# NVIDIAGameWorks/RayTracingDenoiser

Hardware: AMD Instinct MI355X
Metric: Mpixels/s REBLUR_DIFFUSE_SPECULAR @1440p (higher is better)
Workload: dtype f32

## Files before the change

raytracingdenoiser_amd/csrc/hip/kernels_reblur_spatial.hip:

```cpp
#include "passes.h"
#include "reblur_device.h"

namespace nrdhip {

constexpr int TILE_X = 32;
constexpr int TILE_Y = 8;

__global__ __launch_bounds__(256) void ReblurClassifyTilesKernel(Plane viewZ, Plane tiles, float viewZScale, float denoisingRange, int tilesPerRow, int tileRows) {
    const int wave = threadIdx.x >> 6, lane = threadIdx.x & 63;
    const int tileIndex = blockIdx.x * 4 + wave;
    if (tileIndex >= tilesPerRow * tileRows)
        return;
    const int tx = tileIndex % tilesPerRow, ty = tileIndex / tilesPerRow;
    const int x = tx * 16 + (lane & 3) * 4, y = ty * 16 + (lane >> 2);

    bool allSky = true;
    if (y < viewZ.h && x + 3 < viewZ.w) {
        float4 z = *(const float4*)TexelPtr<const float>(viewZ, x, y);
        allSky = Abs(z.x * viewZScale) > denoisingRange && Abs(z.y * viewZScale) > denoisingRange && Abs(z.z * viewZScale) > denoisingRange && Abs(z.w * viewZScale) > denoisingRange;
    } else {
        for (int i = 0; i < 4; i++) {
            float z = InBounds(viewZ, x + i, y) ? LoadR32F(viewZ, x + i, y) : 0.0f;
            allSky = allSky && Abs(z * viewZScale) > denoisingRange;
        }
// ... 24 lines not shown
    float viewZ, roughness, materialID, NoV, frustumSize;
    float3 N, Nv, Xv, Vv;
    float4 rotator;
    float2 data1;
    float3 geo;
    int cbX0, cbX1;
    float2 wc;
};

struct TapGuides {
    float w;
    float3 Ns, Xvs;
    float NvXvs;
    float roughnessS, materialIDs, zs;
    int2 ts;
    float2 uv;
};

template <int FR, bool NEED_ROUGHNESS>
NRD_D TapGuides FetchTapGuidesFullRect(const ReblurCB& c, const SpatialCtx& s, float2 k, const NormalRoughnessGuide& gIn_Normal_Roughness, const Plane& gIn_ViewPos, bool compareMaterials) {
    TapGuides t;
    const float2 rectSize = ToF2(c.gRectSize), rectSizeInv = ToF2(c.gRectSizeInv);
    const float cxf = __builtin_amdgcn_fmed3f(k.x, 0.0f, rectSize.x - 1.0f), cyf = __builtin_amdgcn_fmed3f(k.y, 0.0f, rectSize.y - 1.0f);
    t.w = (cxf == k.x && cyf == k.y) ? 1.0f : 0.0f;
    t.ts = make_int2((int)cxf, (int)cyf);
    const bool materials = FR == 1 && compareMaterials;
    uint32_t bits = 0u;
    {
        const uint32_t offset = TexelOffset(gIn_ViewPos, t.ts.x, t.ts.y, 16u, true);
        const float4 g = *(const float4*)(gIn_ViewPos.ptr + offset);
        t.Ns = Xyz(g);
        t.zs = g.w;
        if (NEED_ROUGHNESS || FR == 1)
            bits = *(const uint32_t*)(gIn_Normal_Roughness.word.ptr + (offset >> 2));
    }
    const float2 uvc = (k + 0.5f) * rectSizeInv;
    t.Xvs = ReconstructViewPosition(uvc, ToF4(c.gFrustum), t.zs, 0.0f);
    t.NvXvs = t.zs * (k.x * s.geo.x + (k.y * s.geo.y + s.geo.z));
    t.materialIDs = 0.0f;
    if (materials)
        t.materialIDs = DecodedMaterialID(bits);
    t.roughnessS = NEED_ROUGHNESS ? DecodedRoughness(bits) : 0.0f;
    t.uv = k;
    return t;
}

template <SpatialMode MODE, bool CB, int FR, bool NEED_ROUGHNESS>
NRD_D TapGuides FetchTapGuides(const ReblurCB& c, const SpatialCtx& s, float2 uv, const Plane& gIn_Signal, const Plane& gIn_ViewZ, const NormalRoughnessGuide& gIn_Normal_Roughness, const Plane& gIn_ViewPos,
    uint32_t checkerboardMode, uint32_t n, bool compareMaterials) {
    const float2 rectSize = ToF2(c.gRectSize), rectSizeInv = ToF2(c.gRectSizeInv);
    uv = Floor(uv * rectSize);
    if (FR)
        return FetchTapGuidesFullRect<FR, NEED_ROUGHNESS>(c, s, uv, gIn_Normal_Roughness, gIn_ViewPos, compareMaterials);
    TapGuides t;
    uv = uv + 0.5f;
    if (MODE == PRE_BLUR && CB)
        uv = ApplyCheckerboardShift(uv, checkerboardMode, n, c.gFrameIndex);
    const float2 k = uv - 0.5f;
    uv = uv * rectSizeInv;
    const float2 resolutionScale = ToF2(c.gResolutionScale);
    const float2 uvMax = resolutionScale - ToF2(c.gResourceSizeInv) * 0.5f;
    float2 uvScaled = F2(Min(uv.x * resolutionScale.x, uvMax.x), Min(uv.y * resolutionScale.y, uvMax.y));
    const int2 tz = NearestTexel(gIn_ViewZ, uvScaled);
    t.ts = tz;
    if (MODE == PRE_BLUR && CB && checkerboardMode != 2)
        t.ts = NearestTexel(gIn_Signal, F2(uvScaled.x * 0.5f, uvScaled.y));
    t.zs = UnpackViewZ(c, LoadR32F(gIn_ViewZ, tz.x, tz.y));
    float4 Ns = LoadDecodedNormalRoughness(gIn_Normal_Roughness, tz.x, tz.y, t.materialIDs);
// ... 1 lines not shown
    t.roughnessS = Ns.w;
    t.Xvs = ReconstructViewPosition(uv, ToF4(c.gFrustum), t.zs, NRD_ORTHO_MODE(c));
    t.NvXvs = t.zs * (k.x * s.geo.x + (k.y * s.geo.y + s.geo.z));
    t.w = IsInScreenNearest(uv);
    t.uv = uv;
    return t;
}

template <bool PERF>
NRD_D float PoissonGaussianWeight(int n) {
    if (PERF)
        return n < 3 ? REBLUR_GAUSSIAN_WEIGHT_Z1 : REBLUR_GAUSSIAN_WEIGHT_Z03;
    return n < 4 ? REBLUR_GAUSSIAN_WEIGHT_Z1 : REBLUR_GAUSSIAN_WEIGHT_Z05;
}

template <SpatialMode MODE, bool PERF, int KIND, bool SH, bool CB, int FR>
NRD_D typename ReblurSignal<KIND>::type DiffuseSpatialFilterTaps(const ReblurCB& c, const SpatialCtx& s, typename ReblurSignal<KIND>::type diff, const Plane& gIn_Diff, const Plane& gIn_ViewZ,
    const NormalRoughnessGuide& gIn_Normal_Roughness, const Plane& gIn_ViewPos, float4& diffSh, const Plane& gIn_DiffSh, float& sum) {
    typedef ReblurSignal<KIND> Sig;
    constexpr bool OCC = KIND == SIGNAL_OCCLUSION;
    typedef typename Sig::type S;

    float fractionScale = 1.0f, radiusScale = 1.0f;
    if (MODE == PRE_BLUR)
        fractionScale = REBLUR_PRE_BLUR_FRACTION_SCALE;
    else if (MODE == BLUR)
        fractionScale = REBLUR_BLUR_FRACTION_SCALE;
    else {
        radiusScale = REBLUR_POST_BLUR_RADIUS_SCALE;
        fractionScale = REBLUR_POST_BLUR_FRACTION_SCALE;
    }
// ... 24 lines not shown
    float2 hitDistanceWeightParams = GetHitDistanceWeightParams(ExtractHitDist(diff), diffNonLinearAccumSpeed);
    float minHitDistWeight = c.gMinHitDistanceWeight * fractionScale;
    if (MODE != PRE_BLUR && !OCC)
        minHitDistWeight *= Sqrt(diffNonLinearAccumSpeed);

    const float2 rectSizeInv = ToF2(c.gRectSizeInv);

    float2 skew = F2(1.0f, 1.0f);
    if (MODE != PRE_BLUR) {
        skew = Lerp(F2(1.0f - Abs(s.Nv.x), 1.0f - Abs(s.Nv.y)), F2(1.0f, 1.0f), s.NoV);
        skew = Div(skew, Max(skew.x, skew.y));
    }
    skew = skew * (rectSizeInv * blurRadius);
    float4 scaledRotator = ScaleRotator(s.rotator, skew);
    const bool compareMaterials = FR != 2 && c.gDiffMinMaterial < 3.0f;

#pragma unroll
    for (int n = 0; n < (PERF ? 6 : 8); n++) {
        float3 offset = PERF ? F3(g_Special6[n][0], g_Special6[n][1], g_Special6[n][2]) : F3(g_Special8[n][0], g_Special8[n][1], g_Special8[n][2]);
        const float2 uvTap = s.pixelUv + RotateVector(scaledRotator, F2(offset.x, offset.y));
        TapGuides t = FetchTapGuides<MODE, CB, FR, false>(c, s, uvTap, gIn_Diff, gIn_ViewZ, gIn_Normal_Roughness, gIn_ViewPos, c.gDiffCheckerboard, (uint32_t)n, compareMaterials);
        const int2 ts = t.ts;

        float angle = AcosApprox(Dot(s.N, t.Ns));

        float w = t.w;
        w *= ComputeWeight(t.NvXvs, geometryWeightParams.x, geometryWeightParams.y);
        if (compareMaterials)
            w *= CompareMaterials(s.materialID, t.materialIDs, c.gDiffMinMaterial) ? 1.0f : 0.0f;
        w *= ComputeWeight(angle, normalWeightParam, 0.0f);

        S smp = Sig::LoadOrZero(gIn_Diff, ts.x, ts.y, w == 0.0f);

        w *= Lerp(minHitDistWeight, 1.0f, ComputeExponentialWeight(ExtractHitDist(smp), hitDistanceWeightParams.x, hitDistanceWeightParams.y));
        w *= PoissonGaussianWeight<PERF>(n);

        sum += w;
        diff = Mad(smp, w, diff);
        if (SH) {
            float4 sh = LoadRGBA16F(gIn_DiffSh, ts.x, ts.y);
            sh = Select(w == 0.0f, F4(0.0f), sh);
            diffSh = Mad(sh, w, diffSh);
        }
    }

    float invSum = PositiveRcp(sum);
    if (SH)
        diffSh = diffSh * invSum;
    return diff * invSum;
}

template <SpatialMode MODE, bool PERF, int KIND, bool SH, bool CB, int FR>
NRD_D typename ReblurSignal<KIND>::type DiffuseSpatialFilter(const ReblurCB& c, const SpatialCtx& s, typename ReblurSignal<KIND>::type diff, const Plane& gIn_Diff, const Plane& gIn_ViewZ,
    const NormalRoughnessGuide& gIn_Normal_Roughness, const Plane& gIn_ViewPos, float4& diffSh, const Plane& gIn_DiffSh, float sum) {
    typedef ReblurSignal<KIND> Sig;
    typedef typename Sig::type S;
    if (!(MODE == PRE_BLUR && c.gDiffPrepassBlurRadius == 0.0f))
        diff = DiffuseSpatialFilterTaps<MODE, PERF, KIND, SH, CB, FR>(c, s, diff, gIn_Diff, gIn_ViewZ, gIn_Normal_Roughness, gIn_ViewPos, diffSh, gIn_DiffSh, sum);
    if (MODE == PRE_BLUR && CB && sum == 0.0f) {
        S s0 = Select(s.wc.x == 0.0f, Sig::Zero(), Sig::Load(gIn_Diff, s.cbX0, s.py));
        S s1 = Select(s.wc.y == 0.0f, Sig::Zero(), Sig::Load(gIn_Diff, s.cbX1, s.py));
        diff = s0 * s.wc.x + s1 * s.wc.y;
        if (SH) {
            float4 sh0 = Select(s.wc.x == 0.0f, F4(0.0f), LoadRGBA16F(gIn_DiffSh, s.cbX0, s.py));
            float4 sh1 = Select(s.wc.y == 0.0f, F4(0.0f), LoadRGBA16F(gIn_DiffSh, s.cbX1, s.py));
            diffSh = sh0 * s.wc.x + sh1 * s.wc.y;
        }
    }
    return diff;
}

template <SpatialMode MODE, bool PERF, int KIND, bool SH, bool CB, int FR>
NRD_D typename ReblurSignal<KIND>::type SpecularSpatialFilterTaps(const ReblurCB& c, const SpatialCtx& s, typename ReblurSignal<KIND>::type spec, const Plane& gIn_Spec, const Plane& gIn_ViewZ,
    const NormalRoughnessGuide& gIn_Normal_Roughness, const Plane& gIn_ViewPos, const Plane& gOut_SpecHitDistForTracking, float4& specSh, const Plane& gIn_SpecSh, float& sum) {
    typedef ReblurSignal<KIND> Sig;
    constexpr bool OCC = KIND == SIGNAL_OCCLUSION;
    typedef typename Sig::type S;
    float smc = GetSpecMagicCurve(s.roughness);

    RngHash rng;
    if (MODE == PRE_BLUR)
        rng.Initialize((uint32_t)s.px, (uint32_t)s.py, c.gFrameIndex);

    float fractionScale = 1.0f, radiusScale = 1.0f;
    if (MODE == PRE_BLUR)
        fractionScale = REBLUR_PRE_BLUR_FRACTION_SCALE;
    else if (MODE == BLUR)
// ... 34 lines not shown
    }
    blurRadius *= radiusScale;
    blurRadius = Max(blurRadius, c.gMinBlurRadius * smc);

    float roughnessFractionScaled = Sat(c.gRoughnessFraction * fractionScale);
    float2 geometryWeightParams = GetGeometryWeightParams(c.gPlaneDistSensitivity, s.frustumSize, s.Xv, s.Nv);
    float normalWeightParam = Div(GetNormalWeightParam(specNonLinearAccumSpeed, c.gLobeAngleFraction, s.roughness), fractionScale);
    float2 roughnessWeightParams = GetRoughnessWeightParams(s.roughness, roughnessFractionScaled);
    float2 hitDistanceWeightParams = GetHitDistanceWeightParams(ExtractHitDist(spec), specNonLinearAccumSpeed, s.roughness);
    float minHitDistWeight = c.gMinHitDistanceWeight * fractionScale * smc;
    if (MODE != PRE_BLUR && !OCC)
        minHitDistWeight *= Sqrt(specNonLinearAccumSpeed);

    const float2 rectSizeInv = ToF2(c.gRectSizeInv);
    const bool compareMaterials = FR != 2 && c.gSpecMinMaterial < 3.0f;

    constexpr bool SCREEN_SPACE = MODE == PRE_BLUR || PERF;
    float4 scaledRotator = F4(0.0f);
    float3 T = F3(0.0f), B = F3(0.0f);
    if (SCREEN_SPACE) {
        float2 skew = rectSizeInv * blurRadius;
        scaledRotator = ScaleRotator(s.rotator, skew);
    } else {
        float bentFactor = Sqrt(hitDistFactor);
        float skewFactor = Lerp(0.25f + 0.75f * s.roughness, 1.0f, NoD);
        skewFactor = Lerp(skewFactor, 1.0f, specNonLinearAccumSpeed);
        skewFactor = Lerp(1.0f, skewFactor, bentFactor);
        float3 bentDv = Normalize(Lerp(s.Nv, Xyz(Dv), bentFactor));
        GetKernelBasis(bentDv, s.Nv, T, B);
        float worldRadius = PixelRadiusToWorld(c.gUnproject, NRD_ORTHO_MODE(c), blurRadius, s.viewZ);
        T = T * (worldRadius * skewFactor);
        B = B * (Div(worldRadius, skewFactor));
    }
    KernelProjection kernelProjection = {};
    if (!SCREEN_SPACE)
        kernelProjection = MakeKernelProjection(c.gViewToClip, s.Xv, T, B, s.rotator);

#pragma unroll
    for (int n = 0; n < (PERF ? 6 : 8); n++) {
        float3 offset = PERF ? F3(g_Special6[n][0], g_Special6[n][1], g_Special6[n][2]) : F3(g_Special8[n][0], g_Special8[n][1], g_Special8[n][2]);
        float2 uv;
        if (SCREEN_SPACE)
            uv = s.pixelUv + RotateVector(scaledRotator, F2(offset.x, offset.y));
        else
            uv = KernelSampleUv(kernelProjection, offset.x, offset.y);
        TapGuides t = FetchTapGuides<MODE, CB, FR, true>(c, s, uv, gIn_Spec, gIn_ViewZ, gIn_Normal_Roughness, gIn_ViewPos, c.gSpecCheckerboard, (uint32_t)n, compareMaterials);
        const int2 ts = t.ts;
        const float zs = t.zs;
        const float3 Xvs = t.Xvs;
        const float4 Ns = F4(t.Ns, t.roughnessS);

        float angle = AcosApprox(Dot(s.N, t.Ns));

        float w = t.w;
        w *= ComputeWeight(t.NvXvs, geometryWeightParams.x, geometryWeightParams.y);
        if (compareMaterials)
            w *= CompareMaterials(s.materialID, t.materialIDs, c.gSpecMinMaterial) ? 1.0f : 0.0f;
        w *= ComputeWeight(angle, normalWeightParam, 0.0f);
        w *= ComputeWeight(Ns.w, roughnessWeightParams.x, roughnessWeightParams.y);

        S smp = Sig::LoadOrZero(gIn_Spec, ts.x, ts.y, w == 0.0f);

        if (MODE == PRE_BLUR) {
            float hs = ExtractHitDist(smp) * GetHitDistanceNormalization(zs, hitDistParams, Ns.w);
            float d = Length(Xvs - s.Xv) + NRD_EPS;
            float geometryWeight = w * Sat(Div(hs, d));
            if (rng.GetFloat() < geometryWeight)
                hitDistForTracking = Min(hitDistForTracking, hs);

            w *= c.gUsePrepassNotOnlyForSpecularMotionEstimation;

            float t = Div(hs, d + hitDist);
            w *= Lerp(Sat(t), 1.0f, LinearStep(0.5f, 1.0f, s.roughness));
        }
        w *= Lerp(minHitDistWeight, 1.0f, ComputeExponentialWeight(ExtractHitDist(smp), hitDistanceWeightParams.x, hitDistanceWeightParams.y));
        w *= PoissonGaussianWeight<PERF>(n);

        sum += w;
        spec = Mad(smp, w, spec);
        if (SH) {
            float4 sh = LoadRGBA16F(gIn_SpecSh, ts.x, ts.y);
            sh = Select(w == 0.0f, F4(0.0f), sh);
            specSh.x += sh.x * w, specSh.y += sh.y * w, specSh.z += sh.z * w;
        }
    }

    float invSum = PositiveRcp(sum);
    spec = spec * invSum;
    if (SH)
        specSh.x *= invSum, specSh.y *= invSum, specSh.z *= invSum;

    if (MODE == PRE_BLUR)
        StoreR16F(gOut_SpecHitDistForTracking, s.px, s.py, hitDistForTracking == NRD_INF ? 0.0f : hitDistForTracking);
    return spec;
}

template <SpatialMode MODE, bool PERF, int KIND, bool SH, bool CB, int FR>
NRD_D typename ReblurSignal<KIND>::type SpecularSpatialFilter(const ReblurCB& c, const SpatialCtx& s, typename ReblurSignal<KIND>::type spec, const Plane& gIn_Spec, const Plane& gIn_ViewZ,
    const NormalRoughnessGuide& gIn_Normal_Roughness, const Plane& gIn_ViewPos, const Plane& gOut_SpecHitDistForTracking, float4& specSh, const Plane& gIn_SpecSh, float sum) {
    typedef ReblurSignal<KIND> Sig;
    typedef typename Sig::type S;
    if (!(MODE == PRE_BLUR && c.gSpecPrepassBlurRadius == 0.0f))
        spec = SpecularSpatialFilterTaps<MODE, PERF, KIND, SH, CB, FR>(c, s, spec, gIn_Spec, gIn_ViewZ, gIn_Normal_Roughness, gIn_ViewPos, gOut_SpecHitDistForTracking, specSh, gIn_SpecSh, sum);
    if (MODE == PRE_BLUR && CB && sum == 0.0f) {
        S s0 = Select(s.wc.x == 0.0f, Sig::Zero(), Sig::Load(gIn_Spec, s.cbX0, s.py));
        S s1 = Select(s.wc.y == 0.0f, Sig::Zero(), Sig::Load(gIn_Spec, s.cbX1, s.py));
        spec = s0 * s.wc.x + s1 * s.wc.y;
        if (SH) {
            float4 sh0 = Select(s.wc.x == 0.0f, F4(0.0f), LoadRGBA16F(gIn_SpecSh, s.cbX0, s.py));
            float4 sh1 = Select(s.wc.y == 0.0f, F4(0.0f), LoadRGBA16F(gIn_SpecSh, s.cbX1, s.py));
            specSh = sh0 * s.wc.x + sh1 * s.wc.y;
        }
    }
    return spec;
}

NRD_D bool MakeSpatialCtx(const ReblurCB& c, int px, int py, float viewZ, const NormalRoughnessGuide& gIn_Normal_Roughness, float4 rotator, SpatialCtx& s) {
    s.viewZ = viewZ;
// ... 22 lines not shown


struct SpatialPlanes {
    Plane tiles, normalRoughness, viewZ, data1;
    NormalRoughnessGuide decodedNR;
    Plane viewPos;
    Plane inDiff, inSpec;
    Plane outDiff, outSpec;
    Plane outHitDistForTracking;
    Plane outViewZ;
    Plane outNormalRoughness;
    Plane outInternalData, outDiffCopy, outSpecCopy;
    Plane inDiffSh, inSpecSh, outDiffSh, outSpecSh, outDiffShCopy, outSpecShCopy;
};

template <SpatialMode MODE, bool DIFF, bool SPEC, bool NO_TS, bool PERF, int KIND, bool SH, bool CB, int FR>
__global__ __launch_bounds__(TILE_X* TILE_Y, NRD_WAVES_REBLUR_SPATIAL) void ReblurSpatialKernel(ReblurCB c, SpatialPlanes P, RowRange rr) {
    typedef ReblurSignal<KIND> Sig;
    constexpr bool OCC = KIND == SIGNAL_OCCLUSION;
    typedef typename Sig::type S;
    const int px = BlockTileX(rr) * TILE_X + (threadIdx.x % TILE_X);
    const int py = (BlockTileY(rr, NRD_ALT_TILE_ORDER && MODE == BLUR)) * TILE_Y + (threadIdx.x / TILE_X);
    if (px > c.gRectSizeMinusOne.x || py > c.gRectSizeMinusOne.y || py < rr.rowBegin || py >= rr.rowEnd)
        return;
    if (LoadR8Unorm(P.tiles, px >> 4, py >> 4) != 0.0f)
        return;

    const float viewZpacked = LoadR32F(P.viewZ, px, py);
    if (MODE == BLUR)
        StoreR32F(P.outViewZ, px, py, viewZpacked);

    SpatialCtx s;
// ... 24 lines not shown
            StoreR16U(P.outInternalData, px, py, PackInternalData(s.data1.x + 1.0f, s.data1.y + 1.0f, s.materialID));
    }

    if (DIFF) {
        const int pos = (MODE == PRE_BLUR && CB && c.gDiffCheckerboard != 2) ? px >> 1 : px;
        float sum = 1.0f;
        S diff = Sig::Load(P.inDiff, pos, py);
        float4 diffSh = F4(0.0f);
        if (SH)
            diffSh = LoadRGBA16F(P.inDiffSh, pos, py);
        if (MODE == PRE_BLUR && CB && c.gDiffCheckerboard != 2 && checkerboard != c.gDiffCheckerboard) {
            sum = 0.0f;
            diff = Sig::Zero();
            diffSh = F4(0.0f);
        }
        diff = DiffuseSpatialFilter<MODE, PERF, KIND, SH, CB, FR>(c, s, diff, P.inDiff, P.viewZ, P.decodedNR, P.viewPos, diffSh, P.inDiffSh, sum);
        Sig::Store(P.outDiff, px, py, diff);
        if (SH)
            StoreRGBA16F(P.outDiffSh, px, py, diffSh);
        if (MODE == POST_BLUR && NO_TS && !OCC)
            Sig::Store(P.outDiffCopy, px, py, diff);
        if (MODE == POST_BLUR && NO_TS && SH)
            StoreRGBA16F(P.outDiffShCopy, px, py, diffSh);
    }
    if (SPEC) {
        const int pos = (MODE == PRE_BLUR && CB && c.gSpecCheckerboard != 2) ? px >> 1 : px;
        float sum = 1.0f;
        S spec = Sig::Load(P.inSpec, pos, py);
        float4 specSh = F4(0.0f);
        if (SH)
            specSh = LoadRGBA16F(P.inSpecSh, pos, py);
        if (MODE == PRE_BLUR && CB && c.gSpecCheckerboard != 2 && checkerboard != c.gSpecCheckerboard) {
            sum = 0.0f;
            spec = Sig::Zero();
            specSh = F4(0.0f);
        }
        spec = SpecularSpatialFilter<MODE, PERF, KIND, SH, CB, FR>(c, s, spec, P.inSpec, P.viewZ, P.decodedNR, P.viewPos, P.outHitDistForTracking, specSh, P.inSpecSh, sum);
        Sig::Store(P.outSpec, px, py, spec);
        if (SH)
            StoreRGBA16F(P.outSpecSh, px, py, specSh);
        if (MODE == POST_BLUR && NO_TS && !OCC)
            Sig::Store(P.outSpecCopy, px, py, spec);
        if (MODE == POST_BLUR && NO_TS && SH)
            StoreRGBA16F(P.outSpecShCopy, px, py, specSh);
    }
}

static bool ForceGenericTaps() {
    const char* v = getenv("NRD_HIP_GENERIC_TAPS");
    return v && atoi(v) != 0;
}

static const char* CheckSupported(const ReblurCB& c) {
    if (c.gRectOrigin.x != 0 || c.gRectOrigin.y != 0)
        return "internal error: a pass was handed a non-zero rectOrigin";
    if (c.gOrthoMode != 0.0f)
        return "REBLUR: orthographic projection is not supported (SURVEY.md section 8c)";
    return nullptr;
}

template <SpatialMode MODE, bool DIFF, bool SPEC, bool NO_TS, bool PERF, int KIND, bool SH>
static const char* LaunchSpatial(const PassArgs& a) {
    constexpr bool OCC = KIND == SIGNAL_OCCLUSION;
    const ReblurCB& c = *(const ReblurCB*)a.constants;
    if (const char* err = CheckSupported(c))
// ... 40 lines not shown
                if (SPEC && !OCC) P.outSpecCopy = a.planes[k++];
                if (DIFF && SH) P.outDiffShCopy = a.planes[k++];
                if (SPEC && SH) P.outSpecShCopy = a.planes[k++];
            }
            if (DIFF && SH) P.outDiffSh = a.planes[k++];
            if (SPEC && SH) P.outSpecSh = a.planes[k++];
        }
    }
    if (k != a.planesNum)
        return "REBLUR spatial pass: unexpected resource count";

    RowGrid g = GridForRows(c.gRectSizeMinusOne.x + 1, c.gRectSizeMinusOne.y + 1, TILE_X, TILE_Y, a.rowBegin, a.rowEnd);
    const RowRange rows = MakeRowRange(g);
    if constexpr (MODE == PRE_BLUR) {
        if (c.gDiffCheckerboard != 2 || c.gSpecCheckerboard != 2) {
            LaunchPass(a, (ReblurSpatialKernel<MODE, DIFF, SPEC, NO_TS, PERF, KIND, SH, true, 0>), g.grid, dim3(TILE_X * TILE_Y), c, P, rows);
            return nullptr;
        }
    }
    const bool fullRect = c.gResolutionScale.x == 1.0f && c.gResolutionScale.y == 1.0f && c.gRectSizeMinusOne.x + 1 == P.decodedNR.nz.w &&
                          c.gRectSizeMinusOne.y + 1 == P.decodedNR.nz.h && P.viewZ.w == P.decodedNR.nz.w && P.viewZ.h == P.decodedNR.nz.h && !ForceGenericTaps();
    const bool materials = (DIFF && c.gDiffMinMaterial < 3.0f) || (SPEC && c.gSpecMinMaterial < 3.0f);
    if (fullRect && !materials)
        LaunchPass(a, (ReblurSpatialKernel<MODE, DIFF, SPEC, NO_TS, PERF, KIND, SH, false, 2>), g.grid, dim3(TILE_X * TILE_Y), c, P, rows);
    else if (fullRect)
        LaunchPass(a, (ReblurSpatialKernel<MODE, DIFF, SPEC, NO_TS, PERF, KIND, SH, false, 1>), g.grid, dim3(TILE_X * TILE_Y), c, P, rows);
    else
        LaunchPass(a, (ReblurSpatialKernel<MODE, DIFF, SPEC, NO_TS, PERF, KIND, SH, false, 0>), g.grid, dim3(TILE_X * TILE_Y), c, P, rows);
    return nullptr;
}

template <bool DIFF, bool SPEC, int KIND>
__global__ __launch_bounds__(256) void ReblurSplitScreenKernel(ReblurCB c, Plane viewZ, Plane inDiff, Plane inSpec, Plane outDiff, Plane outSpec, Plane inDiffSh, Plane inSpecSh, Plane outDiffSh,
    Plane outSpecSh, RowRange rr) {
    const int px = BlockTileX(rr) * TILE_X + (threadIdx.x % TILE_X);
    const int py = (BlockTileY(rr)) * TILE_Y + (threadIdx.x / TILE_X);
    if (px > c.gRectSizeMinusOne.x || py > c.gRectSizeMinusOne.y || py < rr.rowBegin || py >= rr.rowEnd)
        return;
    float pixelUvX = (float(px) + 0.5f) * c.gRectSizeInv.x;
    if (pixelUvX > c.gSplitScreen)
        return;
    float z = UnpackViewZ(c, LoadR32F(viewZ, px, py));
    float keep = z < c.gDenoisingRange ? 1.0f : 0.0f;
// ... 195 lines not shown
```

raytracingdenoiser_amd/csrc/hip/planes.h:

```cpp
#pragma once

#include <hip/hip_fp16.h>
#include <hip/hip_runtime.h>

#include <cstdint>
#include <type_traits>

namespace nrdhip {

struct Plane {
    uint8_t* ptr;
    uint32_t pitch;
    int32_t w, h;
};

#define NRD_D __device__ __forceinline__

NRD_D void ShareLayout(Plane& p, const Plane& ref) {
    p.pitch = ref.pitch;
    p.w = ref.w;
    p.h = ref.h;
}
NRD_D void ShareSize(Plane& p, const Plane& ref) {
    p.w = ref.w;
// ... 5 lines not shown
NRD_D bool InBounds(const Plane& p, int x, int y) { return (unsigned)x < (unsigned)p.w && (unsigned)y < (unsigned)p.h; }

#ifndef NRD_EXPERIMENT_L1_RESIDENT
#define NRD_EXPERIMENT_L1_RESIDENT 0
#endif
NRD_D uint32_t TexelOffset(const Plane& p, int x, int y, uint32_t bytesPerTexel, bool isLoad) {
    if (NRD_EXPERIMENT_L1_RESIDENT == 2 && isLoad)
        return 0u;
    if (NRD_EXPERIMENT_L1_RESIDENT && isLoad)
        return __umul24((uint32_t)(p.h >> 1) + ((uint32_t)y & 1u), p.pitch) + (((uint32_t)x * bytesPerTexel) & 127u);
    return __umul24((uint32_t)y, p.pitch) + (uint32_t)x * bytesPerTexel;
}
template <typename T>
NRD_D T* TexelPtr(const Plane& p, int x, int y) {
    return (T*)(p.ptr + TexelOffset(p, x, y, (uint32_t)sizeof(T), std::is_const<T>::value));
}

NRD_D float DivSmallIntByConst(float k, float c, float rcpC) {
    float q0 = k * rcpC;
    float r = __builtin_fmaf(-q0, c, k);
    return __builtin_fmaf(r, rcpC, q0);
}
#define NRD_DIV_1023(k) DivSmallIntByConst(k, 1023.0f, 0.0009775171056389809f)
#define NRD_DIV_255(k) DivSmallIntByConst(k, 255.0f, 0.003921568859368563f)
#define NRD_DIV_32767(k) DivSmallIntByConst(k, 32767.0f, 3.0518509447574615e-05f)
#define NRD_DIV_65535(k) DivSmallIntByConst(k, 65535.0f, 1.5259021893143654e-05f)
#define NRD_DIV_127(k) DivSmallIntByConst(k, 127.0f, 0.007874015718698502f)
#define NRD_DIV_63(k) DivSmallIntByConst(k, 63.0f, 0.01587301678955555f)
#define NRD_DIV_15(k) DivSmallIntByConst(k, 15.0f, 0.06666667014360428f)
#define NRD_DIV_3(k) DivSmallIntByConst(k, 3.0f, 0.3333333432674408f)
// ... 139 lines not shown
```

raytracingdenoiser_amd/csrc/hip/reblur_device.h:

```cpp
#pragma once

#include "../common/pass_constants.h"
#include "nrdmath.h"
#include "planes.h"

#ifndef NRD_ORTHO_MODE
#define NRD_ORTHO_MODE(c) 0.0f
#endif

namespace nrdhip {

typedef nrdc::ReblurConstants ReblurCB;

#define REBLUR_MAX_ACCUM_FRAME_NUM 63.0f
#define REBLUR_MAX_MATERIALID_NUM 15.0f
#define REBLUR_PRE_BLUR_FRACTION_SCALE 2.0f
#define REBLUR_PRE_BLUR_NON_LINEAR_ACCUM_SPEED (1.0f / (1.0f + 10.0f))
#define REBLUR_BLUR_FRACTION_SCALE 1.0f
#define REBLUR_POST_BLUR_FRACTION_SCALE 0.5f
#define REBLUR_POST_BLUR_RADIUS_SCALE 2.0f
#define REBLUR_NORMAL_ULP NRD_NORMAL_ENCODING_ERROR
#define REBLUR_ALMOST_ZERO_ANGLE 0.01745240643728351f
#define REBLUR_FIREFLY_SUPPRESSOR_MAX_RELATIVE_INTENSITY 38.0f
#define REBLUR_FIREFLY_SUPPRESSOR_RADIUS_SCALE 0.1f
// ... 767 lines not shown
struct ReblurSignal;
template <>
struct ReblurSignal<SIGNAL_RADIANCE> {
    typedef float4 type;
    static NRD_D float4 Zero() { return F4(0.0f); }
    static NRD_D float4 Load(const Plane& p, int x, int y) { return LoadRGBA16F(p, x, y); }
    static NRD_D float4 LoadOrZero(const Plane& p, int x, int y, bool zero) {
#if NRD_EXPERIMENT_LEGACY_DENANIFY
        return Select(zero, F4(0.0f), LoadRGBA16F(p, x, y));
#endif
        uint2 raw = *TexelPtr<const uint2>(p, x, y);
        raw.x = zero ? 0u : raw.x;
        raw.y = zero ? 0u : raw.y;
        return F4(HalfBitsToFloat((uint16_t)(raw.x & 0xFFFFu)), HalfBitsToFloat((uint16_t)(raw.x >> 16)), HalfBitsToFloat((uint16_t)(raw.y & 0xFFFFu)), HalfBitsToFloat((uint16_t)(raw.y >> 16)));
    }
    static NRD_D void Store(const Plane& p, int x, int y, float4 v) { StoreRGBA16F(p, x, y, v); }
    static NRD_D float4 WithHitDist(float4 s, float hitDist) { return F4(s.x, s.y, s.z, hitDist); }
    static NRD_D float4 FetchHistory(const HistoryFilter& h, const Plane& tex) { return FetchHistoryRGBA16F(h, tex); }
    static NRD_D float LoadFast(const Plane& p, int x, int y) { return LoadR16F(p, x, y); }
    static NRD_D void StoreFast(const Plane& p, int x, int y, float v) { StoreR16F(p, x, y, v); }
    static NRD_D float FetchFastBilinear(const HistoryFilter& h, const Plane& tex) { return FetchHistoryBilinearR16F(h, tex); }
    typedef HistoryTexelsRGBA16F HistoryTexels;
    typedef BilinearTexelsR16F FastTexels;
    static NRD_D void PrefetchHistory(const HistoryFilter& h, const Plane& tex, HistoryTexels& t, bool enable) {
        t.loaded = false;
        t.a = t.b0 = t.b1 = t.c0 = t.c1 = t.d = Raw4{0u, 0u, 0u, 0u};
        if (enable)
            PrefetchHistoryRGBA16F(h, tex, t);
    }
    static NRD_D float4 FetchHistory(const HistoryFilter& h, const Plane& tex, const HistoryTexels& t) { return FetchHistoryRGBA16F(h, tex, t); }
// ... 3 lines not shown
NRD_D float FetchHistoryBilinearR16Unorm(const HistoryFilter& h, const Plane& tex) {
    auto at = [&](int x, int y) { return InBounds(tex, x, y) ? LoadR16Unorm(tex, x, y) : 0.0f; };
    float color = at(h.ox, h.oy) * h.bw.x;
    color += at(h.ox + 1, h.oy) * h.bw.y;
    color += at(h.ox, h.oy + 1) * h.bw.z;
    color += at(h.ox + 1, h.oy + 1) * h.bw.w;
    float s = Sum(h.bw);
    return s < 0.0001f ? 0.0f : Div(color, s);
}
template <>
struct ReblurSignal<SIGNAL_OCCLUSION> {
    typedef float type;
    static NRD_D float Zero() { return 0.0f; }
    static NRD_D float Load(const Plane& p, int x, int y) { return LoadR16Unorm(p, x, y); }
    static NRD_D float LoadOrZero(const Plane& p, int x, int y, bool zero) { return zero ? 0.0f : LoadR16Unorm(p, x, y); }
    static NRD_D void Store(const Plane& p, int x, int y, float v) { StoreR16Unorm(p, x, y, v); }
    static NRD_D float WithHitDist(float, float hitDist) { return hitDist; }
    static NRD_D float FetchHistory(const HistoryFilter& h, const Plane& tex) {
        return FetchHistoryGeneric<float>(h, tex, [](const Plane& p, int x, int y) { return LoadR16Unorm(p, x, y); }, 0.0f);
    }
    static NRD_D float LoadFast(const Plane& p, int x, int y) { return LoadR16Unorm(p, x, y); }
    static NRD_D void StoreFast(const Plane& p, int x, int y, float v) { StoreR16Unorm(p, x, y, v); }
    static NRD_D float FetchFastBilinear(const HistoryFilter& h, const Plane& tex) { return FetchHistoryBilinearR16Unorm(h, tex); }
    struct HistoryTexels {};
    struct FastTexels {};
    static NRD_D void PrefetchHistory(const HistoryFilter&, const Plane&, HistoryTexels&, bool) {}
    static NRD_D type FetchHistory(const HistoryFilter& h, const Plane& tex, const HistoryTexels&) { return FetchHistory(h, tex); }
    static NRD_D void PrefetchFast(const HistoryFilter&, const Plane&, FastTexels&) {}
    static NRD_D float FetchFastBilinear(const HistoryFilter& h, const Plane& tex, const FastTexels&) { return FetchFastBilinear(h, tex); }
};
template <>
struct ReblurSignal<SIGNAL_DIRECTIONAL_OCCLUSION> {
    typedef DirOcc type;
    static NRD_D DirOcc Zero() { return MakeDirOcc(F4(0.0f)); }
    static NRD_D DirOcc Load(const Plane& p, int x, int y) { return MakeDirOcc(LoadRGBA16Snorm(p, x, y)); }
    static NRD_D DirOcc LoadOrZero(const Plane& p, int x, int y, bool zero) { return Select(zero, Zero(), Load(p, x, y)); }
    static NRD_D void Store(const Plane& p, int x, int y, DirOcc s) { StoreRGBA16Snorm(p, x, y, s.v); }
    static NRD_D DirOcc WithHitDist(DirOcc s, float hitDist) { return MakeDirOcc(F4(s.v.x, s.v.y, s.v.z, hitDist)); }
    static NRD_D DirOcc FetchHistory(const HistoryFilter& h, const Plane& tex) {
        return MakeDirOcc(FetchHistoryGeneric<float4>(h, tex, [](const Plane& p, int x, int y) { return LoadRGBA16Snorm(p, x, y); }, F4(0.0f)));
    }
    static NRD_D float LoadFast(const Plane& p, int x, int y) { return LoadR16Unorm(p, x, y); }
    static NRD_D void StoreFast(const Plane& p, int x, int y, float v) { StoreR16Unorm(p, x, y, v); }
    static NRD_D float FetchFastBilinear(const HistoryFilter& h, const Plane& tex) { return FetchHistoryBilinearR16Unorm(h, tex); }
    struct HistoryTexels {};
    struct FastTexels {};
    static NRD_D void PrefetchHistory(const HistoryFilter&, const Plane&, HistoryTexels&, bool) {}
    static NRD_D type FetchHistory(const HistoryFilter& h, const Plane& tex, const HistoryTexels&) { return FetchHistory(h, tex); }
    static NRD_D void PrefetchFast(const HistoryFilter&, const Plane&, FastTexels&) {}
    static NRD_D float FetchFastBilinear(const HistoryFilter& h, const Plane& tex, const FastTexels&) { return FetchFastBilinear(h, tex); }
};
// ... 3 lines not shown
```

Measured before the change: 5285.

## Use AMD buffer-resource loads with shared texel index for spatial tap fetches

Adds buffer-resource based loads for the spatial filter taps. A single linear texel index is computed once per tap and shared across the viewPos, normal/roughness, signal and SH planes. Rejected taps get an out-of-range index, so the hardware returns zero instead of needing a select, and the per-plane address arithmetic and 64-bit pointer math are replaced by 32-bit offsets. It also lowers the waves-per-EU bound for pre-blur tap-buffer kernels. The path is limited to diff+spec full-rect cases where every plane's pitch matches and the size fits the index range; otherwise it falls back to the old kernels.

```diff
diff --git a/raytracingdenoiser_amd/csrc/hip/kernels_reblur_spatial.hip b/raytracingdenoiser_amd/csrc/hip/kernels_reblur_spatial.hip
--- a/raytracingdenoiser_amd/csrc/hip/kernels_reblur_spatial.hip
+++ b/raytracingdenoiser_amd/csrc/hip/kernels_reblur_spatial.hip
@@ -62,11 +62,30 @@
     float NvXvs;
     float roughnessS, materialIDs, zs;
     int2 ts;
+    uint32_t index = 0u;
     float2 uv;
 };
 
-template <int FR, bool NEED_ROUGHNESS>
-NRD_D TapGuides FetchTapGuidesFullRect(const ReblurCB& c, const SpatialCtx& s, float2 k, const NormalRoughnessGuide& gIn_Normal_Roughness, const Plane& gIn_ViewPos, bool compareMaterials) {
+struct TapBuffers {
+    TexelBuffer viewPos, word, signal, sh;
+    float pitchTexels;
+};
+template <bool TB, typename Sig>
+NRD_D TapBuffers MakeTapBuffers(const Plane& gIn_ViewPos, const NormalRoughnessGuide& gIn_Normal_Roughness, const Plane& gIn_Signal, const Plane& gIn_Sh) {
+    TapBuffers b = {};
+    if constexpr (TB) {
+        b.viewPos = MakeTexelBuffer(gIn_ViewPos);
+        b.word = MakeTexelBuffer(gIn_Normal_Roughness.word);
+        b.signal = MakeTexelBuffer(gIn_Signal);
+        b.sh = MakeTexelBuffer(gIn_Sh);
+        b.pitchTexels = float(gIn_ViewPos.pitch / 16u);
+    }
+    return b;
+}
+
+template <int FR, bool NEED_ROUGHNESS, bool TB>
+NRD_D TapGuides FetchTapGuidesFullRect(const ReblurCB& c, const SpatialCtx& s, float2 k, const NormalRoughnessGuide& gIn_Normal_Roughness, const Plane& gIn_ViewPos, const TapBuffers& tb,
+    bool compareMaterials) {
     TapGuides t;
     const float2 rectSize = ToF2(c.gRectSize), rectSizeInv = ToF2(c.gRectSizeInv);
     const float cxf = __builtin_amdgcn_fmed3f(k.x, 0.0f, rectSize.x - 1.0f), cyf = __builtin_amdgcn_fmed3f(k.y, 0.0f, rectSize.y - 1.0f);
@@ -74,7 +93,14 @@
     t.ts = make_int2((int)cxf, (int)cyf);
     const bool materials = FR == 1 && compareMaterials;
     uint32_t bits = 0u;
-    {
+    if (TB) {
+        t.index = (uint32_t)__builtin_fmaf(cyf, tb.pitchTexels, cxf);
+        const float4 g = LoadTexel16(tb.viewPos, t.index);
+        t.Ns = Xyz(g);
+        t.zs = g.w;
+        if (NEED_ROUGHNESS || FR == 1)
+            bits = LoadTexel4(tb.word, t.index);
+    } else {
         const uint32_t offset = TexelOffset(gIn_ViewPos, t.ts.x, t.ts.y, 16u, true);
         const float4 g = *(const float4*)(gIn_ViewPos.ptr + offset);
         t.Ns = Xyz(g);
@@ -93,13 +119,13 @@
     return t;
 }
 
-template <SpatialMode MODE, bool CB, int FR, bool NEED_ROUGHNESS>
+template <SpatialMode MODE, bool CB, int FR, bool NEED_ROUGHNESS, bool TB>
 NRD_D TapGuides FetchTapGuides(const ReblurCB& c, const SpatialCtx& s, float2 uv, const Plane& gIn_Signal, const Plane& gIn_ViewZ, const NormalRoughnessGuide& gIn_Normal_Roughness, const Plane& gIn_ViewPos,
-    uint32_t checkerboardMode, uint32_t n, bool compareMaterials) {
+    const TapBuffers& tb, uint32_t checkerboardMode, uint32_t n, bool compareMaterials) {
     const float2 rectSize = ToF2(c.gRectSize), rectSizeInv = ToF2(c.gRectSizeInv);
     uv = Floor(uv * rectSize);
     if (FR)
-        return FetchTapGuidesFullRect<FR, NEED_ROUGHNESS>(c, s, uv, gIn_Normal_Roughness, gIn_ViewPos, compareMaterials);
+        return FetchTapGuidesFullRect<FR, NEED_ROUGHNESS, TB>(c, s, uv, gIn_Normal_Roughness, gIn_ViewPos, tb, compareMaterials);
     TapGuides t;
     uv = uv + 0.5f;
     if (MODE == PRE_BLUR && CB)
@@ -131,7 +157,7 @@
     return n < 4 ? REBLUR_GAUSSIAN_WEIGHT_Z1 : REBLUR_GAUSSIAN_WEIGHT_Z05;
 }
 
-template <SpatialMode MODE, bool PERF, int KIND, bool SH, bool CB, int FR>
+template <SpatialMode MODE, bool PERF, int KIND, bool SH, bool CB, int FR, bool TB>
 NRD_D typename ReblurSignal<KIND>::type DiffuseSpatialFilterTaps(const ReblurCB& c, const SpatialCtx& s, typename ReblurSignal<KIND>::type diff, const Plane& gIn_Diff, const Plane& gIn_ViewZ,
     const NormalRoughnessGuide& gIn_Normal_Roughness, const Plane& gIn_ViewPos, float4& diffSh, const Plane& gIn_DiffSh, float& sum) {
     typedef ReblurSignal<KIND> Sig;
@@ -186,12 +212,13 @@
     skew = skew * (rectSizeInv * blurRadius);
     float4 scaledRotator = ScaleRotator(s.rotator, skew);
     const bool compareMaterials = FR != 2 && c.gDiffMinMaterial < 3.0f;
+    const TapBuffers tb = MakeTapBuffers<TB, Sig>(gIn_ViewPos, gIn_Normal_Roughness, gIn_Diff, gIn_DiffSh);
 
 #pragma unroll
     for (int n = 0; n < (PERF ? 6 : 8); n++) {
         float3 offset = PERF ? F3(g_Special6[n][0], g_Special6[n][1], g_Special6[n][2]) : F3(g_Special8[n][0], g_Special8[n][1], g_Special8[n][2]);
         const float2 uvTap = s.pixelUv + RotateVector(scaledRotator, F2(offset.x, offset.y));
-        TapGuides t = FetchTapGuides<MODE, CB, FR, false>(c, s, uvTap, gIn_Diff, gIn_ViewZ, gIn_Normal_Roughness, gIn_ViewPos, c.gDiffCheckerboard, (uint32_t)n, compareMaterials);
+        TapGuides t = FetchTapGuides<MODE, CB, FR, false, TB>(c, s, uvTap, gIn_Diff, gIn_ViewZ, gIn_Normal_Roughness, gIn_ViewPos, tb, c.gDiffCheckerboard, (uint32_t)n, compareMaterials);
         const int2 ts = t.ts;
 
         float angle = AcosApprox(Dot(s.N, t.Ns));
@@ -202,7 +229,8 @@
             w *= CompareMaterials(s.materialID, t.materialIDs, c.gDiffMinMaterial) ? 1.0f : 0.0f;
         w *= ComputeWeight(angle, normalWeightParam, 0.0f);
 
-        S smp = Sig::LoadOrZero(gIn_Diff, ts.x, ts.y, w == 0.0f);
+        const uint32_t index = w == 0.0f ? TEXEL_INDEX_NONE : t.index;
+        S smp = TB ? Sig::LoadAt(tb.signal, index) : Sig::LoadOrZero(gIn_Diff, ts.x, ts.y, w == 0.0f);
 
         w *= Lerp(minHitDistWeight, 1.0f, ComputeExponentialWeight(ExtractHitDist(smp), hitDistanceWeightParams.x, hitDistanceWeightParams.y));
         w *= PoissonGaussianWeight<PERF>(n);
@@ -210,8 +238,7 @@
         sum += w;
         diff = Mad(smp, w, diff);
         if (SH) {
-            float4 sh = LoadRGBA16F(gIn_DiffSh, ts.x, ts.y);
-            sh = Select(w == 0.0f, F4(0.0f), sh);
+            const float4 sh = TB ? DecodeRGBA16Float(LoadTexel8(tb.sh, index)) : Select(w == 0.0f, F4(0.0f), LoadRGBA16F(gIn_DiffSh, ts.x, ts.y));
             diffSh = Mad(sh, w, diffSh);
         }
     }
@@ -222,13 +249,13 @@
     return diff * invSum;
 }
 
-template <SpatialMode MODE, bool PERF, int KIND, bool SH, bool CB, int FR>
+template <SpatialMode MODE, bool PERF, int KIND, bool SH, bool CB, int FR, bool TB>
 NRD_D typename ReblurSignal<KIND>::type DiffuseSpatialFilter(const ReblurCB& c, const SpatialCtx& s, typename ReblurSignal<KIND>::type diff, const Plane& gIn_Diff, const Plane& gIn_ViewZ,
     const NormalRoughnessGuide& gIn_Normal_Roughness, const Plane& gIn_ViewPos, float4& diffSh, const Plane& gIn_DiffSh, float sum) {
     typedef ReblurSignal<KIND> Sig;
     typedef typename Sig::type S;
     if (!(MODE == PRE_BLUR && c.gDiffPrepassBlurRadius == 0.0f))
-        diff = DiffuseSpatialFilterTaps<MODE, PERF, KIND, SH, CB, FR>(c, s, diff, gIn_Diff, gIn_ViewZ, gIn_Normal_Roughness, gIn_ViewPos, diffSh, gIn_DiffSh, sum);
+        diff = DiffuseSpatialFilterTaps<MODE, PERF, KIND, SH, CB, FR, TB>(c, s, diff, gIn_Diff, gIn_ViewZ, gIn_Normal_Roughness, gIn_ViewPos, diffSh, gIn_DiffSh, sum);
     if (MODE == PRE_BLUR && CB && sum == 0.0f) {
         S s0 = Select(s.wc.x == 0.0f, Sig::Zero(), Sig::Load(gIn_Diff, s.cbX0, s.py));
         S s1 = Select(s.wc.y == 0.0f, Sig::Zero(), Sig::Load(gIn_Diff, s.cbX1, s.py));
@@ -242,7 +269,7 @@
     return diff;
 }
 
-template <SpatialMode MODE, bool PERF, int KIND, bool SH, bool CB, int FR>
+template <SpatialMode MODE, bool PERF, int KIND, bool SH, bool CB, int FR, bool TB>
 NRD_D typename ReblurSignal<KIND>::type SpecularSpatialFilterTaps(const ReblurCB& c, const SpatialCtx& s, typename ReblurSignal<KIND>::type spec, const Plane& gIn_Spec, const Plane& gIn_ViewZ,
     const NormalRoughnessGuide& gIn_Normal_Roughness, const Plane& gIn_ViewPos, const Plane& gOut_SpecHitDistForTracking, float4& specSh, const Plane& gIn_SpecSh, float& sum) {
     typedef ReblurSignal<KIND> Sig;
@@ -307,6 +334,7 @@
 
     const float2 rectSizeInv = ToF2(c.gRectSizeInv);
     const bool compareMaterials = FR != 2 && c.gSpecMinMaterial < 3.0f;
+    const TapBuffers tb = MakeTapBuffers<TB, Sig>(gIn_ViewPos, gIn_Normal_Roughness, gIn_Spec, gIn_SpecSh);
 
     constexpr bool SCREEN_SPACE = MODE == PRE_BLUR || PERF;
     float4 scaledRotator = F4(0.0f);
@@ -337,7 +365,7 @@
             uv = s.pixelUv + RotateVector(scaledRotator, F2(offset.x, offset.y));
         else
             uv = KernelSampleUv(kernelProjection, offset.x, offset.y);
-        TapGuides t = FetchTapGuides<MODE, CB, FR, true>(c, s, uv, gIn_Spec, gIn_ViewZ, gIn_Normal_Roughness, gIn_ViewPos, c.gSpecCheckerboard, (uint32_t)n, compareMaterials);
+        TapGuides t = FetchTapGuides<MODE, CB, FR, true, TB>(c, s, uv, gIn_Spec, gIn_ViewZ, gIn_Normal_Roughness, gIn_ViewPos, tb, c.gSpecCheckerboard, (uint32_t)n, compareMaterials);
         const int2 ts = t.ts;
         const float zs = t.zs;
         const float3 Xvs = t.Xvs;
@@ -352,7 +380,8 @@
         w *= ComputeWeight(angle, normalWeightParam, 0.0f);
         w *= ComputeWeight(Ns.w, roughnessWeightParams.x, roughnessWeightParams.y);
 
-        S smp = Sig::LoadOrZero(gIn_Spec, ts.x, ts.y, w == 0.0f);
+        const uint32_t index = w == 0.0f ? TEXEL_INDEX_NONE : t.index;
+        S smp = TB ? Sig::LoadAt(tb.signal, index) : Sig::LoadOrZero(gIn_Spec, ts.x, ts.y, w == 0.0f);
 
         if (MODE == PRE_BLUR) {
             float hs = ExtractHitDist(smp) * GetHitDistanceNormalization(zs, hitDistParams, Ns.w);
@@ -372,8 +401,7 @@
         sum += w;
         spec = Mad(smp, w, spec);
         if (SH) {
-            float4 sh = LoadRGBA16F(gIn_SpecSh, ts.x, ts.y);
-            sh = Select(w == 0.0f, F4(0.0f), sh);
+            const float4 sh = TB ? DecodeRGBA16Float(LoadTexel8(tb.sh, index)) : Select(w == 0.0f, F4(0.0f), LoadRGBA16F(gIn_SpecSh, ts.x, ts.y));
             specSh.x += sh.x * w, specSh.y += sh.y * w, specSh.z += sh.z * w;
         }
     }
@@ -388,13 +416,13 @@
     return spec;
 }
 
-template <SpatialMode MODE, bool PERF, int KIND, bool SH, bool CB, int FR>
+template <SpatialMode MODE, bool PERF, int KIND, bool SH, bool CB, int FR, bool TB>
 NRD_D typename ReblurSignal<KIND>::type SpecularSpatialFilter(const ReblurCB& c, const SpatialCtx& s, typename ReblurSignal<KIND>::type spec, const Plane& gIn_Spec, const Plane& gIn_ViewZ,
     const NormalRoughnessGuide& gIn_Normal_Roughness, const Plane& gIn_ViewPos, const Plane& gOut_SpecHitDistForTracking, float4& specSh, const Plane& gIn_SpecSh, float sum) {
     typedef ReblurSignal<KIND> Sig;
     typedef typename Sig::type S;
     if (!(MODE == PRE_BLUR && c.gSpecPrepassBlurRadius == 0.0f))
-        spec = SpecularSpatialFilterTaps<MODE, PERF, KIND, SH, CB, FR>(c, s, spec, gIn_Spec, gIn_ViewZ, gIn_Normal_Roughness, gIn_ViewPos, gOut_SpecHitDistForTracking, specSh, gIn_SpecSh, sum);
+        spec = SpecularSpatialFilterTaps<MODE, PERF, KIND, SH, CB, FR, TB>(c, s, spec, gIn_Spec, gIn_ViewZ, gIn_Normal_Roughness, gIn_ViewPos, gOut_SpecHitDistForTracking, specSh, gIn_SpecSh, sum);
     if (MODE == PRE_BLUR && CB && sum == 0.0f) {
         S s0 = Select(s.wc.x == 0.0f, Sig::Zero(), Sig::Load(gIn_Spec, s.cbX0, s.py));
         S s1 = Select(s.wc.y == 0.0f, Sig::Zero(), Sig::Load(gIn_Spec, s.cbX1, s.py));
@@ -447,8 +475,19 @@
     Plane inDiffSh, inSpecSh, outDiffSh, outSpecSh, outDiffShCopy, outSpecShCopy;
 };
 
-template <SpatialMode MODE, bool DIFF, bool SPEC, bool NO_TS, bool PERF, int KIND, bool SH, bool CB, int FR>
-__global__ __launch_bounds__(TILE_X* TILE_Y, NRD_WAVES_REBLUR_SPATIAL) void ReblurSpatialKernel(ReblurCB c, SpatialPlanes P, RowRange rr) {
+#ifndef NRD_WAVES_REBLUR_SPATIAL_TB
+#define NRD_WAVES_REBLUR_SPATIAL_TB -1
+#endif
+template <SpatialMode MODE, bool SH, bool TB>
+constexpr int SpatialWaves() {
+    if (!TB)
+        return NRD_WAVES_REBLUR_SPATIAL;
+    if (NRD_WAVES_REBLUR_SPATIAL_TB >= 0)
+        return NRD_WAVES_REBLUR_SPATIAL_TB;
+    return MODE == PRE_BLUR ? (SH ? 6 : 7) : NRD_WAVES_REBLUR_SPATIAL;
+}
+template <SpatialMode MODE, bool DIFF, bool SPEC, bool NO_TS, bool PERF, int KIND, bool SH, bool CB, int FR, bool TB>
+__global__ __launch_bounds__(TILE_X* TILE_Y, (SpatialWaves<MODE, SH, TB>())) void ReblurSpatialKernel(ReblurCB c, SpatialPlanes P, RowRange rr) {
     typedef ReblurSignal<KIND> Sig;
     constexpr bool OCC = KIND == SIGNAL_OCCLUSION;
     typedef typename Sig::type S;
@@ -503,7 +542,7 @@
             diff = Sig::Zero();
             diffSh = F4(0.0f);
         }
-        diff = DiffuseSpatialFilter<MODE, PERF, KIND, SH, CB, FR>(c, s, diff, P.inDiff, P.viewZ, P.decodedNR, P.viewPos, diffSh, P.inDiffSh, sum);
+        diff = DiffuseSpatialFilter<MODE, PERF, KIND, SH, CB, FR, TB>(c, s, diff, P.inDiff, P.viewZ, P.decodedNR, P.viewPos, diffSh, P.inDiffSh, sum);
         Sig::Store(P.outDiff, px, py, diff);
         if (SH)
             StoreRGBA16F(P.outDiffSh, px, py, diffSh);
@@ -524,7 +563,7 @@
             spec = Sig::Zero();
             specSh = F4(0.0f);
         }
-        spec = SpecularSpatialFilter<MODE, PERF, KIND, SH, CB, FR>(c, s, spec, P.inSpec, P.viewZ, P.decodedNR, P.viewPos, P.outHitDistForTracking, specSh, P.inSpecSh, sum);
+        spec = SpecularSpatialFilter<MODE, PERF, KIND, SH, CB, FR, TB>(c, s, spec, P.inSpec, P.viewZ, P.decodedNR, P.viewPos, P.outHitDistForTracking, specSh, P.inSpecSh, sum);
         Sig::Store(P.outSpec, px, py, spec);
         if (SH)
             StoreRGBA16F(P.outSpecSh, px, py, specSh);
@@ -538,6 +577,19 @@
 static bool ForceGenericTaps() {
     const char* v = getenv("NRD_HIP_GENERIC_TAPS");
     return v && atoi(v) != 0;
+}
+
+#ifndef NRD_TAP_BUFFER_PASSES
+#define NRD_TAP_BUFFER_PASSES 3
+#endif
+static bool TapBuffersFit(const SpatialPlanes& P, uint32_t signalBytes) {
+    const uint32_t pitchTexels = P.viewPos.pitch / 16u;
+    if (P.viewPos.pitch % 16u != 0u || (uint64_t)pitchTexels * (uint32_t)P.viewPos.h >= (1u << 24))
+        return false;
+    if (P.decodedNR.word.pitch != pitchTexels * 4u || P.decodedNR.word.h != P.viewPos.h)
+        return false;
+    auto same = [&](const Plane& p, uint32_t bytes) { return !p.ptr || (p.pitch % bytes == 0u && p.pitch / bytes == pitchTexels && p.h == P.viewPos.h); };
+    return same(P.inDiff, signalBytes) && same(P.inSpec, signalBytes) && same(P.inDiffSh, 8u) && same(P.inSpecSh, 8u);
 }
 
 static const char* CheckSupported(const ReblurCB& c) {
@@ -608,19 +660,27 @@
     const RowRange rows = MakeRowRange(g);
     if constexpr (MODE == PRE_BLUR) {
         if (c.gDiffCheckerboard != 2 || c.gSpecCheckerboard != 2) {
-            LaunchPass(a, (ReblurSpatialKernel<MODE, DIFF, SPEC, NO_TS, PERF, KIND, SH, true, 0>), g.grid, dim3(TILE_X * TILE_Y), c, P, rows);
+            LaunchPass(a, (ReblurSpatialKernel<MODE, DIFF, SPEC, NO_TS, PERF, KIND, SH, true, 0, false>), g.grid, dim3(TILE_X * TILE_Y), c, P, rows);
             return nullptr;
         }
     }
     const bool fullRect = c.gResolutionScale.x == 1.0f && c.gResolutionScale.y == 1.0f && c.gRectSizeMinusOne.x + 1 == P.decodedNR.nz.w &&
                           c.gRectSizeMinusOne.y + 1 == P.decodedNR.nz.h && P.viewZ.w == P.decodedNR.nz.w && P.viewZ.h == P.decodedNR.nz.h && !ForceGenericTaps();
     const bool materials = (DIFF && c.gDiffMinMaterial < 3.0f) || (SPEC && c.gSpecMinMaterial < 3.0f);
-    if (fullRect && !materials)
-        LaunchPass(a, (ReblurSpatialKernel<MODE, DIFF, SPEC, NO_TS, PERF, KIND, SH, false, 2>), g.grid, dim3(TILE_X * TILE_Y), c, P, rows);
+    constexpr bool TAP_BUFFERS = NRD_TAP_BUFFER_LOADS && DIFF && SPEC && ((NRD_TAP_BUFFER_PASSES >> MODE) & 1);
+    if (TAP_BUFFERS && fullRect && TapBuffersFit(P, OCC ? 2u : 8u)) {
+        if constexpr (TAP_BUFFERS) {
+            if (!materials)
+                LaunchPass(a, (ReblurSpatialKernel<MODE, DIFF, SPEC, NO_TS, PERF, KIND, SH, false, 2, true>), g.grid, dim3(TILE_X * TILE_Y), c, P, rows);
+            else
+                LaunchPass(a, (ReblurSpatialKernel<MODE, DIFF, SPEC, NO_TS, PERF, KIND, SH, false, 1, true>), g.grid, dim3(TILE_X * TILE_Y), c, P, rows);
+        }
+    } else if (fullRect && !materials)
+        LaunchPass(a, (ReblurSpatialKernel<MODE, DIFF, SPEC, NO_TS, PERF, KIND, SH, false, 2, false>), g.grid, dim3(TILE_X * TILE_Y), c, P, rows);
     else if (fullRect)
-        LaunchPass(a, (ReblurSpatialKernel<MODE, DIFF, SPEC, NO_TS, PERF, KIND, SH, false, 1>), g.grid, dim3(TILE_X * TILE_Y), c, P, rows);
+        LaunchPass(a, (ReblurSpatialKernel<MODE, DIFF, SPEC, NO_TS, PERF, KIND, SH, false, 1, false>), g.grid, dim3(TILE_X * TILE_Y), c, P, rows);
     else
-        LaunchPass(a, (ReblurSpatialKernel<MODE, DIFF, SPEC, NO_TS, PERF, KIND, SH, false, 0>), g.grid, dim3(TILE_X * TILE_Y), c, P, rows);
+        LaunchPass(a, (ReblurSpatialKernel<MODE, DIFF, SPEC, NO_TS, PERF, KIND, SH, false, 0, false>), g.grid, dim3(TILE_X * TILE_Y), c, P, rows);
     return nullptr;
 }
 
diff --git a/raytracingdenoiser_amd/csrc/hip/planes.h b/raytracingdenoiser_amd/csrc/hip/planes.h
--- a/raytracingdenoiser_amd/csrc/hip/planes.h
+++ b/raytracingdenoiser_amd/csrc/hip/planes.h
@@ -43,6 +43,72 @@
 template <typename T>
 NRD_D T* TexelPtr(const Plane& p, int x, int y) {
     return (T*)(p.ptr + TexelOffset(p, x, y, (uint32_t)sizeof(T), std::is_const<T>::value));
+}
+
+#ifndef NRD_TAP_BUFFER_LOADS
+#define NRD_TAP_BUFFER_LOADS (NRD_EXPERIMENT_L1_RESIDENT == 0)
+#endif
+constexpr uint32_t TEXEL_INDEX_NONE = 1u << 27;
+struct TexelBuffer {
+#ifdef NRD_EMU
+    const uint8_t* ptr;
+    uint32_t bytes;
+#else
+    __amdgpu_buffer_rsrc_t rsrc;
+#endif
+};
+NRD_D TexelBuffer MakeTexelBuffer(const Plane& p) {
+    const uint32_t bytes = p.pitch * (uint32_t)p.h;
+    TexelBuffer b;
+#ifdef NRD_EMU
+    b.ptr = p.ptr;
+    b.bytes = bytes;
+#else
+    b.rsrc = __builtin_amdgcn_make_buffer_rsrc(p.ptr, (short)0, (int)bytes, 0x00020000);
+#endif
+    return b;
+}
+#ifdef NRD_EMU
+template <typename T>
+inline T EmuTexelLoad(const TexelBuffer& b, uint32_t index) {
+    T v;
+    const uint64_t offset = (uint64_t)index * sizeof(T);
+    if (offset < b.bytes)
+        memcpy(&v, b.ptr + offset, sizeof(T));
+    else
+        memset(&v, 0, sizeof(T));
+    return v;
+}
+#endif
+NRD_D float4 LoadTexel16(const TexelBuffer& b, uint32_t index) {
+#ifdef NRD_EMU
+    return EmuTexelLoad<float4>(b, index);
+#else
+    const auto v = __builtin_amdgcn_raw_buffer_load_b128(b.rsrc, index * 16u, 0, 0);
+    return make_float4(__uint_as_float(v[0]), __uint_as_float(v[1]), __uint_as_float(v[2]), __uint_as_float(v[3]));
+#endif
+}
+NRD_D uint2 LoadTexel8(const TexelBuffer& b, uint32_t index) {
+#ifdef NRD_EMU
+    return EmuTexelLoad<uint2>(b, index);
+#else
+    const auto v = __builtin_amdgcn_raw_buffer_load_b64(b.rsrc, index * 8u, 0, 0);
+    return make_uint2(v[0], v[1]);
+#endif
+}
+NRD_D uint32_t LoadTexel4(const TexelBuffer& b, uint32_t index) {
+#ifdef NRD_EMU
+    return EmuTexelLoad<uint32_t>(b, index);
+#else
+    return __builtin_amdgcn_raw_buffer_load_b32(b.rsrc, index * 4u, 0, 0);
+#endif
+}
+NRD_D uint32_t LoadTexel2(const TexelBuffer& b, uint32_t index) {
+#ifdef NRD_EMU
+    return EmuTexelLoad<uint16_t>(b, index);
+#else
+    return __builtin_amdgcn_raw_buffer_load_b16(b.rsrc, index * 2u, 0, 0);
+#endif
 }
 
 NRD_D float DivSmallIntByConst(float k, float c, float rcpC) {
diff --git a/raytracingdenoiser_amd/csrc/hip/reblur_device.h b/raytracingdenoiser_amd/csrc/hip/reblur_device.h
--- a/raytracingdenoiser_amd/csrc/hip/reblur_device.h
+++ b/raytracingdenoiser_amd/csrc/hip/reblur_device.h
@@ -805,6 +805,7 @@
         raw.y = zero ? 0u : raw.y;
         return F4(HalfBitsToFloat((uint16_t)(raw.x & 0xFFFFu)), HalfBitsToFloat((uint16_t)(raw.x >> 16)), HalfBitsToFloat((uint16_t)(raw.y & 0xFFFFu)), HalfBitsToFloat((uint16_t)(raw.y >> 16)));
     }
+    static NRD_D float4 LoadAt(const TexelBuffer& b, uint32_t index) { return DecodeRGBA16Float(LoadTexel8(b, index)); }
     static NRD_D void Store(const Plane& p, int x, int y, float4 v) { StoreRGBA16F(p, x, y, v); }
     static NRD_D float4 WithHitDist(float4 s, float hitDist) { return F4(s.x, s.y, s.z, hitDist); }
     static NRD_D float4 FetchHistory(const HistoryFilter& h, const Plane& tex) { return FetchHistoryRGBA16F(h, tex); }
@@ -838,6 +839,7 @@
     static NRD_D float Zero() { return 0.0f; }
     static NRD_D float Load(const Plane& p, int x, int y) { return LoadR16Unorm(p, x, y); }
     static NRD_D float LoadOrZero(const Plane& p, int x, int y, bool zero) { return zero ? 0.0f : LoadR16Unorm(p, x, y); }
+    static NRD_D float LoadAt(const TexelBuffer& b, uint32_t index) { return NRD_DIV_65535(float(LoadTexel2(b, index))); }
     static NRD_D void Store(const Plane& p, int x, int y, float v) { StoreR16Unorm(p, x, y, v); }
     static NRD_D float WithHitDist(float, float hitDist) { return hitDist; }
     static NRD_D float FetchHistory(const HistoryFilter& h, const Plane& tex) {
@@ -859,6 +861,7 @@
     static NRD_D DirOcc Zero() { return MakeDirOcc(F4(0.0f)); }
     static NRD_D DirOcc Load(const Plane& p, int x, int y) { return MakeDirOcc(LoadRGBA16Snorm(p, x, y)); }
     static NRD_D DirOcc LoadOrZero(const Plane& p, int x, int y, bool zero) { return Select(zero, Zero(), Load(p, x, y)); }
+    static NRD_D DirOcc LoadAt(const TexelBuffer& b, uint32_t index) { return MakeDirOcc(DecodeRGBA16Snorm(LoadTexel8(b, index))); }
     static NRD_D void Store(const Plane& p, int x, int y, DirOcc s) { StoreRGBA16Snorm(p, x, y, s.v); }
     static NRD_D DirOcc WithHitDist(DirOcc s, float hitDist) { return MakeDirOcc(F4(s.v.x, s.v.y, s.v.z, hitDist)); }
     static NRD_D DirOcc FetchHistory(const HistoryFilter& h, const Plane& tex) {
```

Result: no change. 5317 (median of 6 runs) (+0.6%).
